# mfalxa/fakepta

Measured on AMD Instinct MI355X. Metric: residual samples/sec (TOA×realization) for 100-psr HD GWB; % FP64 peak, higher is better.
Workload: dtype f64

## Files before the change

### fakepta_amd/csrc/fpta_internal.h

```cpp
#pragma once
#include <hip/hip_runtime.h>
#include <stdint.h>

#include "fused_sched.h"
#include "grid_plan.h"

namespace fpta {

struct SegDesc {
  const double* w;
  const double* amp;
  const double* L;
  const double* LT;
  int32_t lt_ld, lt_rows;
  const uint8_t* mask;
  int64_t w_pstride;
  double idx;
  double freqf;
  int32_t nm;
  int32_t kind;
  int32_t col0;
  int32_t harmonic;
  int32_t l_lower;
  int32_t n_q;
};

struct SynthArgs {
  const int64_t* offs;
  const int32_t* psr_of;
  const double* toas;
  const double* nu;
  const SegDesc* segs;
  int32_t n_seg;
  int32_t P;
  int64_t n_toa;
  const double* coef;
  int32_t K;
  int32_t R_pad;
  double* out;
  int64_t ldo;
  int32_t n_real;
  int32_t accumulate;
  int32_t anchor;
  int32_t w_on;
  const double* w_sigma;
  const int32_t* w_block_of;
  const double* w_esig;
  const double* w_zb;
  int64_t w_nblocks;
  int64_t real0;
  uint32_t k0, k1;
  int64_t coef_len;
  int32_t tile_toa, tile_real;
  double* part;
};

constexpr int kWR = 4;
constexpr int kWT = 2;
constexpr int kWaves = 4;
constexpr int kTileReal = kWR * 16;
constexpr int kTileToa = kWaves * kWT * 16;
constexpr int kRealPad = 128;
constexpr int kMixTiledMinP = 64;

struct ValuVariant {
  int mt, nt;
};
constexpr ValuVariant kValuVariants[] = {{2, 16}, {4, 16}, {4, 8}, {2, 8}, {1, 32}, {1, 16}};
constexpr int kNumValuVariants = sizeof(kValuVariants) / sizeof(kValuVariants[0]);
constexpr ValuVariant kSeededVariants[] = {{1, 16}, {2, 16}, {1, 8}, {2, 8}, {1, 32}, {4, 16}};
static_assert(sizeof(kSeededVariants) == sizeof(kValuVariants), "one variant index selects both tables");

constexpr int kGridMI = 8;
struct GridSegDev {
  const double* ecos;
  const double* esin;
  double* g;
  int32_t nf, half, lde, nm, col0;
  int32_t ntab;
  int32_t nblk;
  const double* tq;
  int32_t ldq, ntq;
};
struct GridSegs {
  GridSegDev s[kGridMaxSeg];
  int32_t n;
};

struct CoefMerge {
  int32_t dst;
  int32_t n;
  int32_t src[kGridMaxSeg];
  int32_t ncol[kGridMaxSeg];
};
hipError_t launch_coef_merge(hipStream_t st, const CoefMerge& m, int32_t P, int32_t K, int32_t R_pad, double* coef);

hipError_t launch_grid_weights(hipStream_t st, const SegDesc& sd, int64_t n_toa, const double* nu,
                               const int32_t* chunk_of, const int32_t* tt_of, const int32_t* row_of,
                               const double* d_of, int32_t w, double beta, int32_t vmax, double* wd,
                               double* dch = nullptr, int32_t s_idx = 0, int32_t n_sig = 1, int32_t half = 0);
hipError_t launch_grid_dft(hipStream_t st, GridSegs gsegs, int32_t P, const double* coef, int32_t K, int32_t R_pad);
hipError_t launch_grid_dft_mfma(hipStream_t st, GridSegs gsegs, int32_t P, const double* coef, int32_t K,
                                int32_t R_pad);
struct DftGenArgs {
  GridSegDev g;
  int32_t n_terms;
  int32_t term_kind[kDftGenTerms];
  int32_t term_seg[kDftGenTerms];
  int32_t term_nm[kDftGenTerms];
  int32_t term_col0[kDftGenTerms];
  const double* term_amp[kDftGenTerms];
  const double* coef;
  int32_t P, K, R_pad, n_real;
  int64_t real0;
  uint32_t k0, k1;
};
hipError_t launch_grid_dft_gen(hipStream_t st, const DftGenArgs& a);

struct GridBand {
  const int4* chunks;
  const int32_t* rows;
  const double* wd;
  const double* g;
  int32_t n_chunks, vmax;
  int64_t grid_rows;
  const int32_t* pgfirst;
  int32_t n_pg;
};
hipError_t launch_grid_interp_mfma(hipStream_t st, const SynthArgs& a, const GridBand& band, int32_t R_pad);
hipError_t launch_grid_interp_ws(hipStream_t st, const SynthArgs& a, const GridBand& band, int32_t R_pad,
                                 bool ws2 = false);
constexpr int kWrReal = 256;
constexpr int kWrBufs = 3;
struct GridWindow {
  const int4* meta;
  const int2* list;
  const int32_t* slot;
};
hipError_t launch_grid_interp_wr(hipStream_t st, const SynthArgs& a, const GridBand& band, const GridWindow& wr,
                                 int32_t R_pad);
hipError_t launch_grid_interp_psr(hipStream_t st, const SynthArgs& a, const GridBand& band, const GridSegDev& gs,
                                  const int32_t* psr_grp, int32_t P, int32_t R_pad);
constexpr int kFusedIW = 4;
constexpr int kFusedNQ = 12;
constexpr int kFusedTerms = 2;
struct FusedSig {
  const double* tq;
  int32_t ldq, ntq, nf, nm;
  int32_t lrow0;
  int32_t n_rc;
  int32_t n_terms;
  int32_t term_kind[kDftGenTerms];
  int32_t term_seg[kDftGenTerms];
  int32_t term_nm[kDftGenTerms];
  int32_t term_col0[kDftGenTerms];
  const double* term_amp[kDftGenTerms];
};
__host__ __device__ __forceinline__ int64_t fused_half_weight_index(int32_t v, int32_t tt) {
  return ((int64_t)((v >> 3) * 4 + (v & 3)) * kFusedHalfTT + tt) * 2 + ((v >> 2) & 1);
}
struct FusedHalf {
  const int4* chunks;
  const int32_t* lrows;
  const double* wd;
  int32_t fq, vmax;
};
constexpr int kFusedMixMaxP = 256;
constexpr int kFusedMixGroup = 112;
struct FusedMix {
  const double* LT;
  const double* amp;
  double* coef;
  int64_t real0;
  uint32_t k0, k1;
  int32_t lt_ld, lt_rows, P, K, col0, R_pad, n_real, n_q, lower, seg, nm;
  int32_t n_tiles;
};
struct FusedArgs {
  FusedSig s[kFusedMaxSig];
  int32_t n_sig;
  int32_t ring_off;
  const int32_t* lrows;
  int32_t fq;
  const int32_t* psr_c0;
  int64_t real0;
  uint32_t k0, k1;
  unsigned long long* prof;
  uint32_t* queue;
  int32_t join_reserve;
  FusedHalf h;
  int32_t cu_pct;
  FusedMix mix;
};
#ifndef FPTA_FUSED_MIX_CU_PCT
#define FPTA_FUSED_MIX_CU_PCT 100
#endif
constexpr int kFusedQueueWords = 10;
constexpr int kFusedMixWord = 9;
#ifndef FPTA_FUSED_JOIN_SAFETY
#define FPTA_FUSED_JOIN_SAFETY 1.5
#endif
constexpr double kFusedJoinSafety = FPTA_FUSED_JOIN_SAFETY;
hipError_t launch_grid_fused(hipStream_t st, const SynthArgs& a, const GridBand& band, const FusedArgs& f,
                             int32_t nq_max, size_t lds_bytes, hipEvent_t ev0 = nullptr, hipEvent_t ev1 = nullptr,
                             bool half = false, int* kernel_out = nullptr, int* shape_out = nullptr);
constexpr int kFusedKernels = 9;
hipError_t launch_grid_interp_st(hipStream_t st, const SynthArgs& a, const GridBand& band, int32_t R_pad);
struct GridLds {
  const int4* groups;
  const int32_t* urows;
  const int32_t* lrows;
  int32_t n_groups, lds_rows;
};
hipError_t launch_grid_interp_lds(hipStream_t st, const SynthArgs& a, const GridBand& band, const GridLds& lds,
                                  int32_t R_pad);
constexpr int kUnionPitch = 130;
struct GridUnion {
  const int4* groups;
  const int32_t* urows;
  const int32_t* cbase;
  const double* dch;
  const int32_t* wrow;
  int32_t n_groups, n_sig;
  int32_t w[kUnionSigMax];
  double hw[kUnionSigMax], beta[kUnionSigMax];
};
hipError_t launch_grid_interp_u(hipStream_t st, const SynthArgs& a, const GridBand& band, const GridUnion& un,
                                int32_t R_pad);
constexpr int kPartSegs = 64;
constexpr int kPartOneSegs = 16, kPartOneRows = 16 * 48;
constexpr int kPartGroup = 16, kPartGroupMax = 16;
hipError_t launch_part_checksums(hipStream_t st, const double* part, int32_t n_rows, int32_t R_pad, int32_t n_real,
                                 double* tmp, double* sums);

hipError_t launch_seeds(hipStream_t st, const SegDesc* segs, int32_t n_seg, const int32_t* psr_of,
                        const double* toas, const double* nu, int64_t n_toa, double4* seeds);
hipError_t launch_synth_valu_seeded(hipStream_t st, const SynthArgs& a, const int4* tiles, int32_t n_tiles,
                                    const double4* seeds, int variant);

hipError_t launch_gen(hipStream_t st, const SegDesc& sd, int32_t seg_id, int32_t P, int32_t n_real,
                      int32_t R_pad, int64_t real0, uint32_t k0, uint32_t k1, const double* zin,
                      int32_t zin_nseg, int32_t zin_nm, double* coef, int32_t K, double* zbuf);
hipError_t launch_mix(hipStream_t st, const SegDesc& sd, int32_t P, int32_t R_pad, const double* zbuf,
                      double* coef, int32_t K, double* x_out);
hipError_t launch_mix_mfma(hipStream_t st, const SegDesc& sd, int32_t P, int32_t R_pad, const double* zbuf,
                           double* coef, int32_t K, double* x_out, int32_t acc_col0 = -1);
constexpr int kGenMixMaxP = 256;
hipError_t launch_gen_mix(hipStream_t st, const SegDesc& sd, int32_t seg_id, int32_t P, int32_t n_real, int32_t R_pad,
                          int64_t real0, uint32_t k0, uint32_t k1, double* coef, int32_t K, int rh = 2, int rb = 32,
                          hipEvent_t ev0 = nullptr, hipEvent_t ev1 = nullptr);
hipError_t launch_mix_tiled(hipStream_t st, const SegDesc& sd, int32_t P, int32_t R_pad, const double* zbuf,
                            double* coef, int32_t K, double* x_out);
hipError_t launch_epoch_normals(hipStream_t st, int64_t n_blocks, int32_t n_real, int64_t real0, uint32_t k0,
                                uint32_t k1, double* zb);
hipError_t launch_white_pairs(hipStream_t st, const double* sigma, const int32_t* block_of, const double* esig,
                              int64_t n_blocks, const double* zb, double* out, int64_t ldo, int64_t n_toa,
                              int32_t n_real, int64_t real0, uint32_t k0, uint32_t k1);
hipError_t launch_synth_direct(hipStream_t st, const SynthArgs& a);
hipError_t launch_synth_mfma(hipStream_t st, const SynthArgs& a, const int4* tiles, int32_t n_tiles);
hipError_t launch_synth_valu(hipStream_t st, const SynthArgs& a, const int4* tiles, int32_t n_tiles, int variant);
hipError_t launch_white(hipStream_t st, const double* sigma, const int32_t* block_of, const double* esig,
                        const double* z, const double* zb, double* out, int64_t ldo, int64_t n_toa,
                        int32_t n_real, int64_t real0, uint32_t k0, uint32_t k1);
hipError_t launch_checksums(hipStream_t st, const double* out, int64_t ldo, int64_t n_toa, int32_t n_real,
                            double* sums);
hipError_t launch_correlations(hipStream_t st, const double* out, int64_t ldo, int32_t n, int32_t P, int32_t n_real,
                               int32_t mode, double* autos, double* parts, int32_t nparts, double* dst);
hipError_t launch_philox(hipStream_t st, int64_t n, const uint32_t* ctr, uint32_t k0, uint32_t k1,
                         uint32_t* out);
hipError_t launch_normals4(hipStream_t st, int64_t n, const uint32_t* words, double* out);

hipError_t launch_cov_basis(hipStream_t st, const double* toas, const double* nu, int64_t n, const double* f,
                            const double* sw, const int32_t* seg_of, const double* seg_idx, const double* seg_freqf,
                            int32_t n_modes, int32_t k_pad, double* GT, int64_t ldn);
hipError_t launch_gemm_tn(hipStream_t st, const double* a, int64_t lda, const double* b, int64_t ldb, bool b_rows,
                          bool b_tri, double* c, int64_t ldc, int64_t m, int64_t n, int32_t k4, int32_t lower,
                          int32_t tile0, int32_t mode, const double* diag);
hipError_t launch_potrf_block(hipStream_t st, double* C, int64_t ldc, int64_t n, int64_t k0, int* info);
hipError_t launch_trsm_panel(hipStream_t st, double* C, int64_t ldc, int64_t n, int64_t k0, double* PT,
                             int64_t ldp);
hipError_t launch_chol_solve(hipStream_t st, const double* C, int64_t ldc, int64_t n, const double* r,
                             const double* white, double* y, double* out);
hipError_t launch_dense_normals(hipStream_t st, int64_t n, int64_t rows, int32_t n_real, int64_t real0, uint32_t k0,
                                uint32_t k1, double* ZT, int64_t ldz);

}
```

### fakepta_amd/csrc/grid.hip

```cpp
#include <hip/hip_runtime.h>
#include <algorithm>
#include <cstdlib>

#include "device_common.h"
#include "fpta_internal.h"
#include "philox.h"

namespace fpta {

typedef double dbl2 __attribute__((ext_vector_type(2)));

__global__ __launch_bounds__(256) void k_grid_weights(SegDesc sd, int64_t n_toa, const double* __restrict__ nu,
                                                      const int32_t* __restrict__ chunk_of,
                                                      const int32_t* __restrict__ tt_of,
                                                      const int32_t* __restrict__ row_of,
                                                      const double* __restrict__ d_of, int32_t w, double beta,
                                                      int32_t vmax, double* __restrict__ wd, dbl2* __restrict__ dch,
                                                      int32_t s_idx, int32_t n_sig, int32_t half) {
  const int64_t t = (int64_t)blockIdx.x * 256 + threadIdx.x;
  if (t >= n_toa) return;
  double ch = chrom_factor(sd.freqf, nu[t], sd.idx);
  if (sd.mask && !sd.mask[t]) ch = 0.0;
  const double d = d_of[t];
  const double hw = 0.5 * (double)w;
  if (half) {
    double* dst = wd + (int64_t)chunk_of[t] * vmax * kFusedHalfTT;
    for (int i = 0; i < w; ++i) dst[fused_half_weight_index(row_of[t] + i, tt_of[t])] = es_weight(d, i, hw, beta, ch);
    return;
  }
  double* dst = wd + ((int64_t)chunk_of[t] * vmax + row_of[t]) * kGridTT + tt_of[t];
  for (int i = 0; i < w; ++i) dst[(int64_t)i * kGridTT] = es_weight(d, i, hw, beta, ch);
  if (dch) dch[((int64_t)chunk_of[t] * n_sig + s_idx) * kGridTT + tt_of[t]] = dbl2{d, ch};
}

template <int MI>
__global__ __launch_bounds__(256) void k_grid_dft(GridSegs gsegs, const double* __restrict__ coef, int32_t K,
                                                  int32_t R_pad) {
  int bz = blockIdx.z, s = 0;
  while (s + 1 < gsegs.n && bz >= gsegs.s[s].nblk) bz -= gsegs.s[s++].nblk;
  const GridSegDev& gs = gsegs.s[s];
  const int wave = __builtin_amdgcn_readfirstlane(threadIdx.x >> 6);
  const int lane = threadIdx.x & 63;
  const int j0 = bz * MI;
  const int rblk = blockIdx.x * 4 + wave;
  if (rblk * 128 >= R_pad) return;
  const int p = blockIdx.y;
  const int r = rblk * 128 + 2 * lane;
  const double* __restrict__ cp = coef + ((int64_t)p * K + gs.col0) * R_pad + r;
  dbl2 C[MI], S[MI];
#pragma unroll
  for (int i = 0; i < MI; ++i) {
    C[i] = (dbl2){0.0, 0.0};
    S[i] = (dbl2){0.0, 0.0};
  }
  const double* __restrict__ ec = gs.ecos + j0;
  const double* __restrict__ es = gs.esin + j0;
  dbl2 bc0 = *(const dbl2*)cp, bs0 = *(const dbl2*)(cp + R_pad);
  dbl2 bc1 = *(const dbl2*)(cp + 2 * (int64_t)R_pad), bs1 = *(const dbl2*)(cp + 3 * (int64_t)R_pad);
  for (int m = 0; m < gs.nm; m += 2) {
    const int mn = m + 2 < gs.nm ? m + 2 : 0;
    const double* __restrict__ cn = cp + (int64_t)(2 * mn) * R_pad;
    const dbl2 bc0n = *(const dbl2*)cn, bs0n = *(const dbl2*)(cn + R_pad);
    const double* __restrict__ ecm = ec + (int64_t)m * gs.lde;
    const double* __restrict__ esm = es + (int64_t)m * gs.lde;
#pragma unroll
    for (int i = 0; i < MI; ++i) {
      C[i].x = fma(ecm[i], bc0.x, C[i].x);
      C[i].y = fma(ecm[i], bc0.y, C[i].y);
      S[i].x = fma(esm[i], bs0.x, S[i].x);
      S[i].y = fma(esm[i], bs0.y, S[i].y);
    }
    const dbl2 bc1n = *(const dbl2*)(cn + 2 * (int64_t)R_pad), bs1n = *(const dbl2*)(cn + 3 * (int64_t)R_pad);
#pragma unroll
    for (int i = 0; i < MI; ++i) {
      C[i].x = fma(ecm[gs.lde + i], bc1.x, C[i].x);
      C[i].y = fma(ecm[gs.lde + i], bc1.y, C[i].y);
      S[i].x = fma(esm[gs.lde + i], bs1.x, S[i].x);
      S[i].y = fma(esm[gs.lde + i], bs1.y, S[i].y);
    }
    bc0 = bc0n;
    bs0 = bs0n;
    bc1 = bc1n;
    bs1 = bs1n;
  }
  double* __restrict__ gp = gs.g + (int64_t)p * gs.nf * R_pad + r;
#pragma unroll
  for (int i = 0; i < MI; ++i) {
    const int j = j0 + i;
    if (j <= gs.half) *(dbl2*)(gp + (int64_t)j * R_pad) = C[i] + S[i];
    if (j > 0 && 2 * j < gs.nf) *(dbl2*)(gp + (int64_t)(gs.nf - j) * R_pad) = C[i] - S[i];
  }
}

hipError_t launch_grid_weights(hipStream_t st, const SegDesc& sd, int64_t n_toa, const double* nu,
                               const int32_t* chunk_of, const int32_t* tt_of, const int32_t* row_of,
                               const double* d_of, int32_t w, double beta, int32_t vmax, double* wd, double* dch,
                               int32_t s_idx, int32_t n_sig, int32_t half) {
  if (half && (vmax % 8 != 0 || dch)) return hipErrorInvalidValue;
  hipLaunchKernelGGL(k_grid_weights, dim3((unsigned)((n_toa + 255) / 256)), dim3(256), 0, st, sd, n_toa, nu,
                     chunk_of, tt_of, row_of, d_of, w, beta, vmax, wd, (dbl2*)dch, s_idx, n_sig, half);
  return hipGetLastError();
}

hipError_t launch_grid_dft(hipStream_t st, GridSegs gsegs, int32_t P, const double* coef, int32_t K, int32_t R_pad) {
  if (R_pad % 128 != 0 || gsegs.n <= 0 || gsegs.n > kGridMaxSeg) return hipErrorInvalidValue;
  int64_t gx = 0;
  for (int s = 0; s < gsegs.n; ++s) {
    GridSegDev& g = gsegs.s[s];
    if (g.lde < (g.half + kGridMI) / kGridMI * kGridMI || g.nm % 2) return hipErrorInvalidValue;
    g.nblk = (g.half + 1 + kGridMI - 1) / kGridMI;
    gx += g.nblk;
  }
  if (gx > 65535) return hipErrorInvalidValue;
  hipLaunchKernelGGL((k_grid_dft<kGridMI>), dim3((unsigned)((R_pad / 128 + 3) / 4), (unsigned)P, (unsigned)gx), dim3(256),
                     0, st, gsegs, coef, K, R_pad);
  return hipGetLastError();
}

}
```

### fakepta_amd/csrc/grid_fused.hip

```cpp
#include <hip/hip_runtime.h>
#include <hip/hip_ext.h>
#include <algorithm>
#include <atomic>
#include <type_traits>

#include "fused_device.h"

namespace fpta {

#ifndef FPTA_FUSED_DFT_PRIO
#define FPTA_FUSED_DFT_PRIO 3
#endif
#ifndef FPTA_HALF_STORE16
#define FPTA_HALF_STORE16 0
#endif
#ifndef FPTA_HALF_AHEAD
#define FPTA_HALF_AHEAD 2
#endif
constexpr int kFusedHalfAhead = FPTA_HALF_AHEAD;
#ifndef FPTA_HALF_PIN
#define FPTA_HALF_PIN 0
#endif

#ifndef FPTA_FUSED_CUT
// ... 44 lines not shown
  }
  d4 acc[NT][2];
#pragma unroll
  for (int t = 0; t < NT; ++t) acc[t][0] = acc[t][1] = d4{0.0, 0.0, 0.0, 0.0};
  const double* __restrict__ lt = m.LT + p0 + lr;
  const bool paired = (m.real0 & 1) == 0;
  const int e = lr & 1;
  const uint32_t ctr3 = (uint32_t)(g >> 1);
  for (int q0 = 0; q0 < qmax; q0 += 8) {
    double a0[NT], a1[NT];
#pragma unroll
    for (int t = 0; t < NT; ++t) {
      a0[t] = q0 < qe[t] ? ld_global(lt + (int64_t)(q0 + lg) * m.lt_ld + 16 * t) : 0.0;
      a1[t] = q0 + 4 < qe[t] ? ld_global(lt + (int64_t)(q0 + 4 + lg) * m.lt_ld + 16 * t) : 0.0;
    }
    double zc0, zs0, zc1, zs1;
    if (paired) {
      const u32x4 v = philox4x32_10({(uint32_t)k, (uint32_t)(q0 + 4 * e + lg), (uint32_t)m.seg, ctr3}, m.k0, m.k1);
      const uint32_t r0 = dpp_u32_xor1(e ? v.x : v.z), r1 = dpp_u32_xor1(e ? v.y : v.w);
      bm_half(e ? r0 : v.x, e ? r1 : v.y, zc0, zs0);
      bm_half(e ? v.z : r0, e ? v.w : r1, zc1, zs1);
    } else {
      gp_normal2((uint32_t)k, (uint32_t)(q0 + lg), (uint32_t)m.seg, g, m.k0, m.k1, zc0, zs0);
      gp_normal2((uint32_t)k, (uint32_t)(q0 + 4 + lg), (uint32_t)m.seg, g, m.k0, m.k1, zc1, zs1);
    }
    const bool ok0 = rv && q0 + lg < m.n_q, ok1 = rv && q0 + 4 + lg < m.n_q;
    zc0 = ok0 ? zc0 : 0.0;
    zs0 = ok0 ? zs0 : 0.0;
    zc1 = ok1 ? zc1 : 0.0;
    zs1 = ok1 ? zs1 : 0.0;
#pragma unroll
    for (int t = 0; t < NT; ++t)
      if (q0 < qe[t]) {
        acc[t][0] = __builtin_amdgcn_mfma_f64_16x16x4f64(a0[t], zc0, acc[t][0], 0, 0, 0);
        acc[t][1] = __builtin_amdgcn_mfma_f64_16x16x4f64(a0[t], zs0, acc[t][1], 0, 0, 0);
      }
#pragma unroll
    for (int t = 0; t < NT; ++t)
      if (q0 + 4 < qe[t]) {
        acc[t][0] = __builtin_amdgcn_mfma_f64_16x16x4f64(a1[t], zc1, acc[t][0], 0, 0, 0);
        acc[t][1] = __builtin_amdgcn_mfma_f64_16x16x4f64(a1[t], zs1, acc[t][1], 0, 0, 0);
      }
  }
  const double am = ld_global(m.amp + k);
#pragma unroll
  for (int t = 0; t < NT; ++t)
#pragma unroll
    for (int h = 0; h < 2; ++h)
#pragma unroll
      for (int gg = 0; gg < 4; ++gg) {
        const int p = p0 + 16 * t + lg + 4 * gg;
        if (p < m.P) m.coef[((int64_t)p * m.K + m.col0 + 2 * k + h) * m.R_pad + r] = am * acc[t][h][gg];
      }
}

}

template <int NQ, bool ODD, bool GEN, bool HALF, int SHAPE>
__device__ __forceinline__ void grid_fused_body(const SynthArgs& a, const GridBand& band, const FusedArgs& f,
                                                int32_t n_rb, int32_t n_items) {
  static_assert(kFusedTerms == 2 && kFusedMaxSig == 2, "fused_shape_slot's slots and signals (c0, c1)");
  static_assert(SHAPE == kFusedShapeAny || GEN == (SHAPE == kFusedShapeGenLoad), "a shape fixes whether terms are drawn");
  static_assert(kFusedReal == 32 && kFusedPitch == 32 && kFusedGroupModes * kFusedReal / 2 == 64 * kFusedDW,
                "two realization tiles; one (mode, realization pair) of a 16-mode group per DFT lane");
  static_assert(!HALF || (NQ % 4 == 0 && kGridTT == 2 * kFusedHalfTT), "half bands: whole row groups, two halves");
  extern __shared__ __attribute__((aligned(16))) double lds[];
  const FusedQueue queue(n_items, f.queue);
  const int wave = __builtin_amdgcn_readfirstlane(threadIdx.x >> 6);
  const int lane = threadIdx.x & 63;
  const int lr = lane & 15, lg = lane >> 4;
  double* __restrict__ ring = lds + f.ring_off;
  uint32_t* sync = (uint32_t*)(ring + 2 * kFusedMaxSig * kFusedSlot);
  volatile int* qitem = (volatile int*)(sync + 4);
  if (threadIdx.x == 0) {
    *sync = 0u;
    ((volatile int*)sync)[8] = 0;
    ((volatile int*)sync)[9] = 0;
    qitem[0] = queue.fetch();
    qitem[1] = qitem[0] >= 0 ? queue.fetch() : -1;
  }
  __syncthreads();
  auto item_of = [&](int k) { return __builtin_amdgcn_readfirstlane(qitem[k & 3]); };
  auto finish = [&]() {
    if (threadIdx.x == 0) {
      __threadfence();
      const uint32_t done = __hip_atomic_fetch_add(f.queue + 8, 1u, __ATOMIC_ACQ_REL, __HIP_MEMORY_SCOPE_AGENT);
      if (done == gridDim.x - 1)
        for (int i = 0; i < kFusedQueueWords; ++i)
          __hip_atomic_store(f.queue + i, 0u, __ATOMIC_RELAXED, __HIP_MEMORY_SCOPE_AGENT);
    }
  };
  auto mix_tiles = [&]() {
    if (f.mix.n_tiles <= 0) return;
    __builtin_amdgcn_s_setprio(0);
    const int n_pg = (f.mix.P + kFusedMixGroup - 1) / kFusedMixGroup, n_rg = f.mix.R_pad >> 4;
    for (;;) {
      int t = 0;
      if (lane == 0)
        t = (int)__hip_atomic_fetch_add(f.queue + kFusedMixWord, 1u, __ATOMIC_RELAXED, __HIP_MEMORY_SCOPE_AGENT);
      t = __builtin_amdgcn_readfirstlane(t);
      if (t >= f.mix.n_tiles) break;
      const int pg = t % n_pg, kr = t / n_pg;
      const int k = kr / n_rg;
      fused_mix_tile(f.mix, k, kr - k * n_rg, pg, lane);
    }
  };
  if (item_of(0) < 0) {
    finish();
    return;
  }

  volatile int* ccnt = (volatile int*)(sync + 8);
  struct Geo {
    int p, r0, c0, n;
    int64_t toa0;
    bool valid;
  };
  auto geo = [&](int k) {
    Geo g;
    const int item = item_of(k);
    g.valid = item >= 0;
    const int it = g.valid ? item : 0;
    g.p = it / n_rb;
    g.r0 = (it - g.p * n_rb) * kFusedReal;
    g.c0 = ld_uniform(f.psr_c0 + g.p);
    g.n = g.valid ? ld_uniform(f.psr_c0 + g.p + 1) - g.c0 : 0;
    g.toa0 = ld_uniform(a.offs + g.p);
    return g;
  };
  auto ticket = [&](int k) {
    int t = 0;
    if (lane == 0)
      t = __hip_atomic_fetch_add((int*)ccnt + (k & 1), 1, __ATOMIC_RELAXED, __HIP_MEMORY_SCOPE_WORKGROUP);
    return __builtin_amdgcn_readfirstlane(t);
  };
  auto lane_now = [&]() {
    int v = lane;
    asm volatile("" : "+v"(v));
    return v;
  };
  using Ops = typename std::conditional<HALF, FusedOpsH<NQ>, FusedOps<NQ>>::type;
  using OpsJ = typename std::conditional<HALF, FusedOpsH<NQ>, FusedOps<(NQ < 8 ? NQ : 8)>>::type;
  auto load_half = [&](int cc, auto& o, int ln) {
    {
      constexpr int NS = sizeof(o.row[0]) / sizeof(o.row[0][0]);
      o.c = cc;
      o.ci = *(const i32x4*)(f.h.chunks + cc);
      const int lgo = ln >> 4, lro = ln & 15;
#pragma unroll
      for (int h = 0; h < 2; ++h) {
        const i32x4* __restrict__ rt = (const i32x4*)(f.h.lrows + (((int64_t)cc * 2 + h) * 4 + lgo) * f.h.fq);
#pragma unroll
        for (int q4 = 0; q4 < NS / 4; ++q4) {
          const i32x4 r4 = rt[q4];
          o.row[h][4 * q4] = r4.x;
          o.row[h][4 * q4 + 1] = r4.y;
          o.row[h][4 * q4 + 2] = r4.z;
          o.row[h][4 * q4 + 3] = r4.w;
        }
        const double* __restrict__ wp =
            f.h.wd + ((int64_t)cc * 2 + h) * f.h.vmax * kFusedHalfTT + (lgo * kFusedHalfTT + lro) * 2;
#pragma unroll
        for (int qp = 0; qp < NS / 2; ++qp) o.b[h][qp] = *(const dbl2*)(wp + qp * 8 * kFusedHalfTT);
      }
    }
  };
  auto load_full = [&](int cc, auto& o, int ln) {
    constexpr int NS = sizeof(o.row) / sizeof(o.row[0]);
    o.c = cc;
    o.ci = *(const i32x4*)(band.chunks + cc);
    const int lgo = ln >> 4, lro = ln & 15;
    const i32x4* __restrict__ rt = (const i32x4*)(f.lrows + ((int64_t)cc * 4 + lgo) * f.fq);
    const double* __restrict__ wp = band.wd + ((int64_t)cc * band.vmax + lgo) * kGridTT + 2 * lro;
#pragma unroll
    for (int q4 = 0; q4 < NS / 4; ++q4) {
      const i32x4 r4 = rt[q4];
      o.row[4 * q4] = r4.x;
      o.row[4 * q4 + 1] = r4.y;
      o.row[4 * q4 + 2] = r4.z;
      o.row[4 * q4 + 3] = r4.w;
    }
#pragma unroll
    for (int q = 0; q < NS; ++q) o.b[q] = *(const dbl2*)(wp + 4 * kGridTT * q);
  };
  auto load = [&](int cc, auto& o, int ln) {
    if constexpr (HALF)
      load_half(cc, o, ln);
    else
      load_full(cc, o, ln);
  };
  auto process_half = [&](const Geo& g, const auto& cur, auto& pf, int ln) {
    constexpr int NS = sizeof(cur.row[0]) / sizeof(cur.row[0][0]);
    const int lg = ln >> 4, lr = ln & 15;
    const int lds_lane = 2 * lr;
    const int ty = __builtin_amdgcn_readfirstlane(cur.ci.y), tc = __builtin_amdgcn_readfirstlane(cur.ci.z);
    const int nqw = __builtin_amdgcn_readfirstlane(cur.ci.w);
    const int nq[2] = {nqw & 0xFFFF, nqw >> 16};
    FPTA_DCHECK(nq[0] > 0, "k_grid_fused half band steps", nq[0], 1 << 20);
    d4 acc[2][2];
#pragma unroll
    for (int h = 0; h < 2; ++h)
#pragma unroll
      for (int i = 0; i < 2; ++i) acc[h][i] = d4{0.0, 0.0, 0.0, 0.0};
    {
      constexpr int DA = kFusedHalfAhead;
      const int nqm = min(max(nq[0], nq[1]), NS);
      dbl2 an[2][NS];
      auto rd = [&](int q) {
#pragma unroll
        for (int h = 0; h < 2; ++h) an[h][q] = *(const dbl2*)(lds + cur.row[h][q] * kFusedPitch + lds_lane);
      };
#pragma unroll
      for (int q = 0; q < DA && q < NS; ++q) rd(q);
#pragma unroll
      for (int q = 0; q < NS; ++q) {
        if (q < nqm) {
          if (q + DA < NS) rd(q + DA);
          if (FPTA_HALF_PIN) __builtin_amdgcn_sched_barrier(0);
          const double b0 = (q & 1) ? cur.b[0][q >> 1].y : cur.b[0][q >> 1].x;
          const double b1 = (q & 1) ? cur.b[1][q >> 1].y : cur.b[1][q >> 1].x;
          acc[0][0] = __builtin_amdgcn_mfma_f64_16x16x4f64(an[0][q].x, b0, acc[0][0], 0, 0, 0);
          acc[0][1] = __builtin_amdgcn_mfma_f64_16x16x4f64(an[0][q].y, b0, acc[0][1], 0, 0, 0);
          acc[1][0] = __builtin_amdgcn_mfma_f64_16x16x4f64(an[1][q].x, b1, acc[1][0], 0, 0, 0);
          acc[1][1] = __builtin_amdgcn_mfma_f64_16x16x4f64(an[1][q].y, b1, acc[1][1], 0, 0, 0);
        }
      }
    }
    pf.lap(1);
#pragma unroll
    for (int h = 0; h < 2; ++h)
      for (int q = NS; q < nq[h]; ++q) {
        const int64_t hc = (int64_t)cur.c * 2 + h;
        const int row = f.h.lrows[(hc * 4 + lg) * f.h.fq + q];
        const double bv = f.h.wd[hc * f.h.vmax * kFusedHalfTT + fused_half_weight_index(4 * q + lg, lr)];
        const dbl2 av = *(const dbl2*)(lds + row * kFusedPitch + lds_lane);
        acc[h][0] = __builtin_amdgcn_mfma_f64_16x16x4f64(av.x, bv, acc[h][0], 0, 0, 0);
        acc[h][1] = __builtin_amdgcn_mfma_f64_16x16x4f64(av.y, bv, acc[h][1], 0, 0, 0);
      }
    pf.lap(4);
    __builtin_amdgcn_sched_barrier(0);
    const int64_t t0 = g.toa0 + ty;
    if ((FPTA_FUSED_CUT & 8) && acc[0][0][0] != -1.25e300) return;
    if (FPTA_HALF_STORE16 && tc == kGridTT && g.r0 + kFusedReal <= a.n_real && ((t0 | a.ldo) & 1) == 0 &&
        a.ldo < ((int64_t)1 << 26)) {
      const bool odd = lr & 1;
      const uint32_t vo = (uint32_t)(((int64_t)2 * lg * a.ldo + (odd ? 15 + lr : lr)) * 8);
      const char* base = (const char*)(a.out + t0 + (int64_t)g.r0 * a.ldo);
#pragma unroll
      for (int i = 0; i < 2; ++i)
#pragma unroll
        for (int gg = 0; gg < 4; ++gg) {
          const double send = odd ? acc[0][i][gg] : acc[1][i][gg];
          const double recv = dpp_xor1(send);
          const dbl2 v = odd ? dbl2{recv, acc[1][i][gg]} : dbl2{acc[0][i][gg], recv};
          __builtin_nontemporal_store(v, (dbl2*)((char*)base + (int64_t)(8 * gg + i) * a.ldo * 8 + vo));
        }
    } else if (tc == kGridTT && g.r0 + kFusedReal <= a.n_real && a.ldo < ((int64_t)1 << 26)) {
      const uint32_t vo = (uint32_t)(((int64_t)2 * lg * a.ldo + lr) * 8);
      const char* base = (const char*)(a.out + t0 + (int64_t)g.r0 * a.ldo);
#pragma unroll
      for (int h = 0; h < 2; ++h)
#pragma unroll
        for (int i = 0; i < 2; ++i)
#pragma unroll
          for (int gg = 0; gg < 4; ++gg)
            __builtin_nontemporal_store(acc[h][i][gg],
                                        (double*)((char*)base + ((int64_t)(8 * gg + i) * a.ldo + 16 * h) * 8 + vo));
    } else {
#pragma unroll
      for (int h = 0; h < 2; ++h) {
        if (16 * h + lr >= tc) continue;
#pragma unroll
        for (int i = 0; i < 2; ++i)
#pragma unroll
          for (int gg = 0; gg < 4; ++gg) {
            const int r = g.r0 + 2 * (lg + 4 * gg) + i;
            if (r < a.n_real) a.out[t0 + 16 * h + lr + (int64_t)r * a.ldo] = acc[h][i][gg];
          }
      }
    }
    pf.lap(2);
  };
  auto process_full = [&](const Geo& g, const auto& cur, auto& pf, int ln) {
    constexpr int NS = sizeof(cur.row) / sizeof(cur.row[0]);
    const int lg = ln >> 4, lr = ln & 15;
    const int lds_lane = 2 * lr;
    const int ty = __builtin_amdgcn_readfirstlane(cur.ci.y), tc = __builtin_amdgcn_readfirstlane(cur.ci.z);
    const int nq = __builtin_amdgcn_readfirstlane(cur.ci.w) >> 2;
    FPTA_DCHECK(nq > 0, "k_grid_fused band steps", nq, 1 << 20);
    d4 acc[2][2];
#pragma unroll
    for (int e = 0; e < 2; ++e)
#pragma unroll
      for (int i = 0; i < 2; ++i) acc[e][i] = d4{0.0, 0.0, 0.0, 0.0};
    {
      dbl2 an = *(const dbl2*)(lds + cur.row[0] * kFusedPitch + lds_lane);
#pragma unroll
      for (int q = 0; q < NS; ++q) {
        if (q < nq) {
          const dbl2 av = an;
          if (q + 1 < NS) an = *(const dbl2*)(lds + cur.row[q + 1] * kFusedPitch + lds_lane);
          const dbl2 bv = cur.b[q];
          acc[0][0] = __builtin_amdgcn_mfma_f64_16x16x4f64(av.x, bv.x, acc[0][0], 0, 0, 0);
          acc[0][1] = __builtin_amdgcn_mfma_f64_16x16x4f64(av.y, bv.x, acc[0][1], 0, 0, 0);
          acc[1][0] = __builtin_amdgcn_mfma_f64_16x16x4f64(av.x, bv.y, acc[1][0], 0, 0, 0);
          acc[1][1] = __builtin_amdgcn_mfma_f64_16x16x4f64(av.y, bv.y, acc[1][1], 0, 0, 0);
        }
      }
    }
    pf.lap(1);
    for (int q = NS; q < nq; ++q) {
      const int v = 4 * q + lg;
      const int row = f.lrows[((int64_t)cur.c * 4 + lg) * f.fq + q];
      const dbl2 bv = *(const dbl2*)(band.wd + ((int64_t)cur.c * band.vmax + v) * kGridTT + 2 * lr);
      const dbl2 av = *(const dbl2*)(lds + row * kFusedPitch + lds_lane);
      acc[0][0] = __builtin_amdgcn_mfma_f64_16x16x4f64(av.x, bv.x, acc[0][0], 0, 0, 0);
      acc[0][1] = __builtin_amdgcn_mfma_f64_16x16x4f64(av.y, bv.x, acc[0][1], 0, 0, 0);
      acc[1][0] = __builtin_amdgcn_mfma_f64_16x16x4f64(av.x, bv.y, acc[1][0], 0, 0, 0);
      acc[1][1] = __builtin_amdgcn_mfma_f64_16x16x4f64(av.y, bv.y, acc[1][1], 0, 0, 0);
    }
    pf.lap(4);
    __builtin_amdgcn_sched_barrier(0);
    const int64_t t0 = g.toa0 + ty;
    if ((FPTA_FUSED_CUT & 8) && acc[0][0][0] != -1.25e300) return;
    if (FPTA_HALF_STORE16 && tc == kGridTT && g.r0 + kFusedReal <= a.n_real && ((t0 | a.ldo) & 1) == 0 &&
        a.ldo < ((int64_t)1 << 26)) {
      const uint32_t vo = (uint32_t)(((int64_t)2 * lg * a.ldo + 2 * lr) * 8);
      const char* base = (const char*)(a.out + t0 + (int64_t)g.r0 * a.ldo);
#pragma unroll
      for (int i = 0; i < 2; ++i)
#pragma unroll
        for (int gg = 0; gg < 4; ++gg)
          __builtin_nontemporal_store(dbl2{acc[0][i][gg], acc[1][i][gg]},
                                      (dbl2*)((char*)base + (int64_t)(8 * gg + i) * a.ldo * 8 + vo));
    } else {
      InterpTile<2> t;
      t.c = cur.c;
      t.p = g.p;
      t.r0 = g.r0;
      t.y = ty;
      t.cnt = tc;
      t.nq = nq;
      interp_store_rows<2>(a, a.out, t, acc);
    }
    pf.lap(2);
  };
  auto process = [&](const Geo& g, const auto& cur, auto& pf, int ln) {
    if constexpr (HALF)
      process_half(g, cur, pf, ln);
    else
      process_full(g, cur, pf, ln);
  };

  if (wave >= kFusedIW) {
    const int dw = wave - kFusedIW;
    __builtin_amdgcn_s_setprio(FPTA_FUSED_DFT_PRIO);
    constexpr int kNSig = fused_shape_nsig(SHAPE);
    const int n_sig = kNSig ? kNSig : f.n_sig;
    int js = -1, jrc = 0;
    {
      int j = dw;
#pragma unroll
      for (int s = 0; s < kFusedMaxSig; ++s) {
        if (s < n_sig && js < 0 && j < f.s[s].n_rc) {
          js = s;
          jrc = j;
        }
        if (s < n_sig) j -= f.s[s].n_rc;
      }
    }
    js = __builtin_amdgcn_readfirstlane(js);
    jrc = __builtin_amdgcn_readfirstlane(jrc);
    Prof pf;
    pf.start();
    uint32_t epoch = 0;
    auto dsync = [&]() {
      fused_wait_lgkm0();
      if (lane == 0) __hip_atomic_fetch_add(sync, 1u, __ATOMIC_RELAXED, __HIP_MEMORY_SCOPE_WORKGROUP);
      epoch += kFusedDW;
      while ((uint32_t)__builtin_amdgcn_readfirstlane(
                 (int)__hip_atomic_load(sync, __ATOMIC_RELAXED, __HIP_MEMORY_SCOPE_WORKGROUP)) < epoch)
        __builtin_amdgcn_s_sleep(1);
    };
    int ng[kFusedMaxSig];
#pragma unroll
    for (int s = 0; s < kFusedMaxSig; ++s) ng[s] = s < n_sig ? fused_groups(f.s[s].nm) : 0;
    const int n_it = fused_iterations(ng[0], ng[1]);
    const FusedSig& jf = f.s[js < 0 ? 0 : js];
    const int64_t jts = (int64_t)jf.ntq * jf.ldq, jld4 = 4 * (int64_t)jf.ldq;
    auto jtq_now = [&]() {
      const int ln = lane_now();
      return jf.tq + (int64_t)(ln >> 4) * jf.ldq + 32 * jrc + 2 * (ln & 15);
    };
    const int jnq0 = fused_ksteps(jf.nm, 0), jnq1 = fused_ksteps(jf.nm, 1);
    const int jng = js < 0 ? 0 : fused_groups(jf.nm);
    d4 C[2][2][2], S[2][2][2];
    struct DrawIn {
      dbl2 x0[kFusedTerms], x1[kFusedTerms];
    };
    std::integral_constant<int, 0> c0;
    std::integral_constant<int, 1> c1;
    auto draw_load = [&](auto sc, int g, int p, int r0, DrawIn& in) {
      constexpr int s = decltype(sc)::value;
      const FusedSig& fs = f.s[s];
      const int didx = dw * 64 + lane_now(), dmm = didx >> 4, drl = 2 * (didx & 15);
      const int m = kFusedGroupModes * g + dmm, r = r0 + drl;
      auto slot = [&](auto ic) {
        constexpr int i = decltype(ic)::value, kind = fused_shape_slot(SHAPE, s, i);
        if constexpr (kind == kFusedSlotGen) {
          const int nmi = fs.term_nm[i], mi = min(m, nmi - 1);
          in.x0[i] = ld_global((const dbl2*)(fs.term_amp[i] + (int64_t)p * nmi + (mi & ~1)));
        } else if constexpr (kind == kFusedSlotLoad) {
          const int mi = min(m, fs.term_nm[i] - 1);
          const double* src0 = a.coef + ((int64_t)p * a.K + fs.term_col0[i] + 2 * mi) * a.R_pad + r;
          in.x0[i] = ld_global((const dbl2*)src0);
          in.x1[i] = ld_global((const dbl2*)(src0 + a.R_pad));
        } else if constexpr (kind == kFusedSlotAny) {
          const bool on = i < fs.n_terms;
          const int nmi = on ? fs.term_nm[i] : 2;
          const int mi = min(m, nmi - 1);
          const double* src0;
          int64_t step;
          if (on && fs.term_kind[i] == 1) {
            src0 = a.coef + ((int64_t)p * a.K + fs.term_col0[i] + 2 * mi) * a.R_pad + r;
            step = a.R_pad;
          } else {
            src0 = (on ? fs.term_amp[i] : a.coef) + (int64_t)p * nmi + (mi & ~1);
            step = 0;
          }
          in.x0[i] = ld_global((const dbl2*)src0);
          in.x1[i] = ld_global((const dbl2*)(src0 + step));
        }
// ... 433 lines not shown
```

### fakepta_amd/csrc/grid_plan.h

```cpp
#pragma once
#include <algorithm>
#include <cmath>
#include <cstdint>
#include <string>
#include <vector>

namespace fpta {

constexpr int kGridTT = 32;
constexpr int kGridRowCap = 48;
constexpr int kGridVMax = 256;
constexpr int kGridMinV = 16;
constexpr int kGridMaxSeg = 16;
#ifndef FPTA_DFT_MJ
#define FPTA_DFT_MJ 2
#endif
constexpr int kDftMJ = FPTA_DFT_MJ;
constexpr int kDftMR = 4 / FPTA_DFT_MJ;
constexpr int kGridDftRows = 16 * kDftMJ;
constexpr int kDftGenTerms = 8;
constexpr int kFusedMaxSig = 2;
constexpr int kFusedReal = 32;
constexpr int kFusedPitch = 32;
constexpr int kFusedDW = 4;
constexpr int kFusedGroupModes = 16;
constexpr int kFusedSlot = kFusedGroupModes * kFusedReal * 2;
constexpr int kFusedLdsMax = 160 * 1024;
constexpr int kFusedFqMin = 16;
constexpr int kFusedPadRows = 4 * kFusedFqMin;
constexpr int kFusedHalfTT = 16;
constexpr int kFusedHalfNQ = 8;
constexpr int kWrSlots = 32, kWrMaxSig = 2, kWrVMax = 40;
constexpr int kWrFresh = 1 << 30;
constexpr int kWrFar = 1 << 29;
constexpr int kLdsGroup = 4, kLdsRowsMax = 144;
constexpr int kUnionGroup = 4, kUnionRowsMax = 76, kUnionSigMax = 2;

struct Int4 {
  int32_t x, y, z, w;
};

struct PlanSignal {
  int32_t kind = 0, nm = 0;
  double idx = 0.0, freqf = 0.0;
  int32_t harmonic = 0;
  const double* w0 = nullptr;
  const uint8_t* mask = nullptr;
};
struct PlanLayout {
  int32_t P = 0;
  int64_t n_toa = 0;
  const int64_t* offs = nullptr;
  const double* toas = nullptr;
  const double* nu = nullptr;
  std::vector<PlanSignal> sigs;
};
struct PlanOptions {
  int32_t w = 0;
  double sigma = 0.0;
  bool coalesce = false;
  int32_t grid_mfma = 1;
};

struct PlanSeg {
  int32_t nm = 0;
  int32_t nf = 0, w = 0, half = 0, lde = 0, ntab = 0, ldq = 0, ntq = 0;
  double beta = 0.0;
  int64_t rowoff = 0;
  std::vector<double> ecos, esin;
  std::vector<double> tq;
  std::vector<int32_t> row;
  std::vector<double> d;
  std::vector<int32_t> hrow_of;
  std::vector<int64_t> J;
  std::vector<int64_t> band_lo;
  std::vector<int32_t> band_n;
  std::vector<int32_t> voff;
};
struct PlanFigures {
  bool ok = false;
  std::string why;
  std::vector<std::vector<int32_t>> members;
  std::vector<int32_t> anchor, last;
  bool merges = false;
  std::vector<int32_t> psr_chunk0;
  int32_t vmax = 0;
  int64_t grid_rows = 0;
  bool fused_ok = false;
  size_t fused_lds = 0;
  int32_t fused_fq = 0;
  std::vector<int32_t> fused_lrow0;
  bool fused_half_ok = false;
  int32_t fused_hfq = 0, fused_hvmax = 0, fused_hnq = 0;
  double fused_half_gain = 0.0;
  double fma_interp_half = 0.0;
  double mean_v = 0.0;
  double fma_grid = 0.0;
  double fma_dft = 0.0;
  double fma_interp = 0.0;
  double grid_vals = 0.0;
  double weight_bytes = 0.0;
  double fma_direct = 0.0;
  double err_bound = 1.0;
};
struct HostGridPlan : PlanFigures {
  std::vector<PlanSeg> segs;
  std::vector<Int4> chunks;
  std::vector<int32_t> chunk_of, tt_of;
  std::vector<int32_t> rows;
  size_t wd_size = 0;
  std::vector<int32_t> frows;
  std::vector<Int4> hchunks;
  std::vector<int32_t> hrows, hchunk_of, htt_of;
  std::vector<int32_t> hv;
  size_t hwd_size = 0;
  int32_t n_seg() const { return (int32_t)segs.size(); }
  int32_t n_chunks() const { return (int32_t)chunks.size(); }
};

inline int32_t plan_wrap(int64_t j, int32_t nf) { return (int32_t)((j % nf + nf) % nf); }

inline void gauss_legendre(int n, std::vector<double>& x, std::vector<double>& wt) {
  x.assign(n, 0.0);
  wt.assign(n, 0.0);
  for (int i = 0; i < (n + 1) / 2; ++i) {
    double z = std::cos(M_PI * (i + 0.75) / (n + 0.5)), dp = 1.0;
    for (int it = 0; it < 100; ++it) {
      double p0 = 1.0, p1 = z;
      for (int k = 2; k <= n; ++k) {
        const double p2 = ((2.0 * k - 1.0) * z * p1 - (k - 1.0) * p0) / k;
        p0 = p1;
        p1 = p2;
      }
      dp = n * (z * p1 - p0) / (z * z - 1.0);
      const double dz = p1 / dp;
      z -= dz;
      if (std::fabs(dz) < 1e-16) break;
    }
    x[i] = -z;
    x[n - 1 - i] = z;
    wt[i] = wt[n - 1 - i] = 2.0 / ((1.0 - z * z) * dp * dp);
  }
}

inline void plan_coalesce(const PlanLayout& L, const PlanOptions& o, HostGridPlan& H) {
  const int32_t n_layout = (int32_t)L.sigs.size();
  std::vector<std::vector<double>> chv(n_layout);
  auto ch_of = [&](int32_t i) -> const std::vector<double>& {
    if (chv[i].empty()) {
      const PlanSignal& d = L.sigs[i];
      chv[i].resize(L.n_toa);
      for (int64_t t = 0; t < L.n_toa; ++t) {
        double ch = 1.0;
        if (d.idx != 0.0) {
          const double x = d.freqf / L.nu[t];
          ch = d.idx == 2.0 ? x * x : d.idx == 1.0 ? x : std::pow(x, d.idx);
        }
        chv[i][t] = (d.mask && !d.mask[t]) ? 0.0 : ch;
      }
    }
    return chv[i];
  };
  auto w0_of = [&](int32_t i, int32_t p) { return L.sigs[i].w0[L.sigs[i].kind == 0 ? p : 0]; };
  for (int32_t i = 0; i < n_layout; ++i) {
    int32_t join = -1;
    for (size_t g = 0; o.coalesce && g < H.members.size() && join < 0; ++g) {
      if (H.members[g].size() > (size_t)kGridMaxSeg) continue;
      const int32_t f = H.members[g][0];
      bool same = true;
      for (int32_t p = 0; p < L.P && same; ++p) same = w0_of(i, p) == w0_of(f, p);
      if (same) same = ch_of(i) == ch_of(f);
      if (same) join = (int32_t)g;
    }
    if (join < 0) {
      H.members.push_back({i});
    } else {
      H.members[join].push_back(i);
      H.merges = true;
    }
  }
  for (const std::vector<int32_t>& m : H.members) {
    int32_t a = m[0];
    for (int32_t i : m)
      if (L.sigs[i].nm > L.sigs[a].nm) a = i;
// ... 339 lines not shown
```

Before: 393.0 billion.

## Transpose fused half MFMA operands and permute TOA rows for vector stores

The order of the two operands in the f64 MFMA calls is swapped, so the accumulator holds realizations on rows and TOAs on columns. The weight layout gets a TOA-row permutation so that each lane ends up owning consecutive TOA pairs. The epilogue then writes paired dbl2 nontemporal stores along the contiguous TOA axis. This replaces the previous DPP-exchange store path and the strided scalar stores. The goal is fewer, wider global stores, at the cost of added index-permutation logic in the weight build and the fallback store path.

```diff
diff --git a/fakepta_amd/csrc/fpta_internal.h b/fakepta_amd/csrc/fpta_internal.h
--- a/fakepta_amd/csrc/fpta_internal.h
+++ b/fakepta_amd/csrc/fpta_internal.h
@@ -156,9 +156,6 @@
   int32_t term_col0[kDftGenTerms];
   const double* term_amp[kDftGenTerms];
 };
-__host__ __device__ __forceinline__ int64_t fused_half_weight_index(int32_t v, int32_t tt) {
-  return ((int64_t)((v >> 3) * 4 + (v & 3)) * kFusedHalfTT + tt) * 2 + ((v >> 2) & 1);
-}
 struct FusedHalf {
   const int4* chunks;
   const int32_t* lrows;
diff --git a/fakepta_amd/csrc/grid.hip b/fakepta_amd/csrc/grid.hip
--- a/fakepta_amd/csrc/grid.hip
+++ b/fakepta_amd/csrc/grid.hip
@@ -25,7 +25,8 @@
   const double hw = 0.5 * (double)w;
   if (half) {
     double* dst = wd + (int64_t)chunk_of[t] * vmax * kFusedHalfTT;
-    for (int i = 0; i < w; ++i) dst[fused_half_weight_index(row_of[t] + i, tt_of[t])] = es_weight(d, i, hw, beta, ch);
+    const int col = fused_half_toa_row(tt_of[t]);
+    for (int i = 0; i < w; ++i) dst[fused_half_weight_index(row_of[t] + i, col)] = es_weight(d, i, hw, beta, ch);
     return;
   }
   double* dst = wd + ((int64_t)chunk_of[t] * vmax + row_of[t]) * kGridTT + tt_of[t];
diff --git a/fakepta_amd/csrc/grid_fused.hip b/fakepta_amd/csrc/grid_fused.hip
--- a/fakepta_amd/csrc/grid_fused.hip
+++ b/fakepta_amd/csrc/grid_fused.hip
@@ -220,7 +220,7 @@
         const i32x4* __restrict__ rt = (const i32x4*)(f.h.lrows + (((int64_t)cc * 2 + h) * 4 + lgo) * f.h.fq);
 #pragma unroll
         for (int q4 = 0; q4 < NS / 4; ++q4) {
-          const i32x4 r4 = rt[q4];
+          const i32x4 r4 = (FPTA_FUSED_CUT & 16) ? i32x4{4 * q4, 4 * q4 + 1, 4 * q4 + 2, 4 * q4 + 3} : rt[q4];
           o.row[h][4 * q4] = r4.x;
           o.row[h][4 * q4 + 1] = r4.y;
           o.row[h][4 * q4 + 2] = r4.z;
@@ -287,10 +287,10 @@
           if (FPTA_HALF_PIN) __builtin_amdgcn_sched_barrier(0);
           const double b0 = (q & 1) ? cur.b[0][q >> 1].y : cur.b[0][q >> 1].x;
           const double b1 = (q & 1) ? cur.b[1][q >> 1].y : cur.b[1][q >> 1].x;
-          acc[0][0] = __builtin_amdgcn_mfma_f64_16x16x4f64(an[0][q].x, b0, acc[0][0], 0, 0, 0);
-          acc[0][1] = __builtin_amdgcn_mfma_f64_16x16x4f64(an[0][q].y, b0, acc[0][1], 0, 0, 0);
-          acc[1][0] = __builtin_amdgcn_mfma_f64_16x16x4f64(an[1][q].x, b1, acc[1][0], 0, 0, 0);
-          acc[1][1] = __builtin_amdgcn_mfma_f64_16x16x4f64(an[1][q].y, b1, acc[1][1], 0, 0, 0);
+          acc[0][0] = __builtin_amdgcn_mfma_f64_16x16x4f64(b0, an[0][q].x, acc[0][0], 0, 0, 0);
+          acc[0][1] = __builtin_amdgcn_mfma_f64_16x16x4f64(b0, an[0][q].y, acc[0][1], 0, 0, 0);
+          acc[1][0] = __builtin_amdgcn_mfma_f64_16x16x4f64(b1, an[1][q].x, acc[1][0], 0, 0, 0);
+          acc[1][1] = __builtin_amdgcn_mfma_f64_16x16x4f64(b1, an[1][q].y, acc[1][1], 0, 0, 0);
         }
       }
     }
@@ -302,50 +302,44 @@
         const int row = f.h.lrows[(hc * 4 + lg) * f.h.fq + q];
         const double bv = f.h.wd[hc * f.h.vmax * kFusedHalfTT + fused_half_weight_index(4 * q + lg, lr)];
         const dbl2 av = *(const dbl2*)(lds + row * kFusedPitch + lds_lane);
-        acc[h][0] = __builtin_amdgcn_mfma_f64_16x16x4f64(av.x, bv, acc[h][0], 0, 0, 0);
-        acc[h][1] = __builtin_amdgcn_mfma_f64_16x16x4f64(av.y, bv, acc[h][1], 0, 0, 0);
+        acc[h][0] = __builtin_amdgcn_mfma_f64_16x16x4f64(bv, av.x, acc[h][0], 0, 0, 0);
+        acc[h][1] = __builtin_amdgcn_mfma_f64_16x16x4f64(bv, av.y, acc[h][1], 0, 0, 0);
       }
     pf.lap(4);
     __builtin_amdgcn_sched_barrier(0);
     const int64_t t0 = g.toa0 + ty;
     if ((FPTA_FUSED_CUT & 8) && acc[0][0][0] != -1.25e300) return;
-    if (FPTA_HALF_STORE16 && tc == kGridTT && g.r0 + kFusedReal <= a.n_real && ((t0 | a.ldo) & 1) == 0 &&
-        a.ldo < ((int64_t)1 << 26)) {
-      const bool odd = lr & 1;
-      const uint32_t vo = (uint32_t)(((int64_t)2 * lg * a.ldo + (odd ? 15 + lr : lr)) * 8);
-      const char* base = (const char*)(a.out + t0 + (int64_t)g.r0 * a.ldo);
-#pragma unroll
-      for (int i = 0; i < 2; ++i)
-#pragma unroll
-        for (int gg = 0; gg < 4; ++gg) {
-          const double send = odd ? acc[0][i][gg] : acc[1][i][gg];
-          const double recv = dpp_xor1(send);
-          const dbl2 v = odd ? dbl2{recv, acc[1][i][gg]} : dbl2{acc[0][i][gg], recv};
-          __builtin_nontemporal_store(v, (dbl2*)((char*)base + (int64_t)(8 * gg + i) * a.ldo * 8 + vo));
-        }
-    } else if (tc == kGridTT && g.r0 + kFusedReal <= a.n_real && a.ldo < ((int64_t)1 << 26)) {
-      const uint32_t vo = (uint32_t)(((int64_t)2 * lg * a.ldo + lr) * 8);
-      const char* base = (const char*)(a.out + t0 + (int64_t)g.r0 * a.ldo);
+    if (tc == kGridTT && g.r0 + kFusedReal <= a.n_real && ((t0 | a.ldo) & 1) == 0) {
+      char* base = (char*)(a.out + t0 + 2 * lg + (int64_t)(g.r0 + 2 * lr) * a.ldo);
 #pragma unroll
       for (int h = 0; h < 2; ++h)
 #pragma unroll
         for (int i = 0; i < 2; ++i)
 #pragma unroll
+          for (int gp = 0; gp < 2; ++gp)
+            __builtin_nontemporal_store(dbl2{acc[h][i][2 * gp], acc[h][i][2 * gp + 1]},
+                                        (dbl2*)(base + ((int64_t)i * a.ldo + 16 * h + 8 * gp) * 8));
+    } else if (tc == kGridTT && g.r0 + kFusedReal <= a.n_real) {
+      double* base = a.out + t0 + 2 * lg + (int64_t)(g.r0 + 2 * lr) * a.ldo;
+#pragma unroll
+      for (int h = 0; h < 2; ++h)
+#pragma unroll
+        for (int i = 0; i < 2; ++i)
+#pragma unroll
           for (int gg = 0; gg < 4; ++gg)
-            __builtin_nontemporal_store(acc[h][i][gg],
-                                        (double*)((char*)base + ((int64_t)(8 * gg + i) * a.ldo + 16 * h) * 8 + vo));
+            __builtin_nontemporal_store(acc[h][i][gg], base + (int64_t)i * a.ldo + 16 * h + 8 * (gg >> 1) + (gg & 1));
     } else {
 #pragma unroll
-      for (int h = 0; h < 2; ++h) {
-        if (16 * h + lr >= tc) continue;
-#pragma unroll
-        for (int i = 0; i < 2; ++i)
+      for (int h = 0; h < 2; ++h)
+#pragma unroll
+        for (int i = 0; i < 2; ++i) {
+          const int r = g.r0 + 2 * lr + i;
 #pragma unroll
           for (int gg = 0; gg < 4; ++gg) {
-            const int r = g.r0 + 2 * (lg + 4 * gg) + i;
-            if (r < a.n_real) a.out[t0 + 16 * h + lr + (int64_t)r * a.ldo] = acc[h][i][gg];
+            const int tt = 16 * h + fused_half_row_toa(lg + 4 * gg);
+            if (tt < tc && r < a.n_real) a.out[t0 + tt + (int64_t)r * a.ldo] = acc[h][i][gg];
           }
-      }
+        }
     }
     pf.lap(2);
   };
diff --git a/fakepta_amd/csrc/grid_plan.h b/fakepta_amd/csrc/grid_plan.h
--- a/fakepta_amd/csrc/grid_plan.h
+++ b/fakepta_amd/csrc/grid_plan.h
@@ -30,6 +30,17 @@
 constexpr int kFusedPadRows = 4 * kFusedFqMin;
 constexpr int kFusedHalfTT = 16;
 constexpr int kFusedHalfNQ = 8;
+#if defined(__HIPCC__)
+#define FPTA_PLAN_HD __host__ __device__ inline
+#else
+#define FPTA_PLAN_HD inline
+#endif
+FPTA_PLAN_HD int64_t fused_half_weight_index(int32_t v, int32_t tt) {
+  return ((int64_t)((v >> 3) * 4 + (v & 3)) * kFusedHalfTT + tt) * 2 + ((v >> 2) & 1);
+}
+FPTA_PLAN_HD int32_t fused_half_toa_row(int32_t tt) { return ((tt >> 1) & 3) + 4 * (tt & 1) + (tt & 8); }
+FPTA_PLAN_HD int32_t fused_half_row_toa(int32_t m) { return 2 * (m & 3) + ((m >> 2) & 1) + (m & 8); }
+#undef FPTA_PLAN_HD
 constexpr int kWrSlots = 32, kWrMaxSig = 2, kWrVMax = 40;
 constexpr int kWrFresh = 1 << 30;
 constexpr int kWrFar = 1 << 29;
```

Result: slower. 370.2 billion (-5.8%).
